# SCUT-BIP-Lab/SplatCo

Measured on AMD Instinct MI355X. Metric: rasterizer fwd+bwd Msplats/s @1080p; PSNR-match vs ref, higher is better.
Workload: dtype f32; 1 GPU; cfg1: 1M synthetic Gaussians (seed 0), 1 view 1920x1080 per GPU, GaussianRasterizer forward+backward, colors_precomp + scale/rotation path; gaussians=1000000, image=1920x1080, visible=1000000, parallelism=1 view per GPU (mv sharding)

## Files before the change

splatco_amd/csrc/binning.hip:

```cpp
#include "common.h"

namespace scr {

template <int THREADS>
__device__ __forceinline__ uint32_t block_exclusive_scan(uint32_t v, uint32_t* lds_waves ,
                                                         uint32_t& block_total) {
    const int lane = threadIdx.x & (WAVE - 1), w = threadIdx.x / WAVE;
    uint32_t inc = v;
#pragma unroll
    for (int d = 1; d < WAVE; d <<= 1) {
        uint32_t n = __shfl_up(inc, d, WAVE);
        if (lane >= d) inc += n;
    }
    if (lane == WAVE - 1) lds_waves[w] = inc;
    __syncthreads();
    uint32_t base = 0, tot = 0;
#pragma unroll
    for (int k = 0; k < THREADS / WAVE; ++k) {
        uint32_t s = lds_waves[k];
        if (k < w) base += s;
        tot += s;
    }
    block_total = tot;
    __syncthreads();
    return base + inc - v;
}

__global__ void __launch_bounds__(1024) plan_scan_kernel(uint32_t nblk, uint32_t* __restrict__ block_sums,
                                                         unsigned long long* __restrict__ total,
                                                         uint32_t tiles, const uint32_t* __restrict__ tile_count,
                                                         uint32_t* __restrict__ ranges,
                                                         uint32_t* __restrict__ cursor,
                                                         volatile unsigned long long* mailbox,
                                                         unsigned long long seq) {
    __shared__ uint32_t lds[1024 / WAVE + 1];
    __shared__ unsigned long long wide[1024 / WAVE];
    if (blockIdx.x == 0) {
        unsigned long long carry = 0, mine = 0;
        for (uint32_t base = 0; base < nblk; base += 1024) {
            uint32_t i = base + threadIdx.x;
            uint32_t v = i < nblk ? block_sums[i] : 0u, tot;
            uint32_t ex = block_exclusive_scan<1024>(v, lds, tot);
            if (i < nblk) block_sums[i] = (uint32_t)carry + ex;
            carry += tot;
            mine += v;
        }
#pragma unroll
        for (int d = WAVE / 2; d > 0; d >>= 1) mine += (unsigned long long)__shfl_down((long long)mine, d, WAVE);
        __syncthreads();
        if ((threadIdx.x & (WAVE - 1)) == 0) wide[threadIdx.x / WAVE] = mine;
        __syncthreads();
        if (threadIdx.x == 0) {
            carry = 0;
            for (int w = 0; w < 1024 / WAVE; ++w) carry += wide[w];
            total[0] = carry;
            if (mailbox) {
                mailbox[0] = carry;
                __threadfence_system();
                mailbox[1] = seq;
            }
        }
    } else {
        uint32_t carry = 0, mx = 0;
        for (uint32_t base = 0; base < tiles; base += 1024) {
            uint32_t i = base + threadIdx.x;
            uint32_t v = i < tiles ? tile_count[i] : 0u, tot;
            uint32_t ex = block_exclusive_scan<1024>(v, lds, tot);
            if (i < tiles) {
                ranges[2 * i] = carry + ex;
                ranges[2 * i + 1] = carry + ex + v;
                cursor[i] = 0;
            }
            carry += tot;
            mx = max(mx, v);
        }
#pragma unroll
        for (int d = 32; d > 0; d >>= 1) mx = max(mx, (uint32_t)__shfl_xor((int)mx, d, WAVE));
        __syncthreads();
        if ((threadIdx.x & 63) == 0) lds[threadIdx.x >> 6] = mx;
        __syncthreads();
        if (threadIdx.x == 0) {
            uint32_t m = 0;
            for (int w = 0; w < 1024 / WAVE; ++w) m = max(m, lds[w]);
            total[1] = m;
            total[2] = 0;
            if (mailbox) {
                mailbox[2] = (unsigned long long)m | (total[3] << 32);
                __threadfence_system();
                mailbox[3] = seq;
            }
        }
    }
}

template <bool LDS_HIST>
__global__ void __launch_bounds__(BIN_THREADS)
scatter_kernel(int64_t P, int gx, int tiles, const float4* __restrict__ rec, uint2* __restrict__ gm_base,
               uint32_t* __restrict__ live_bits, const uint32_t* __restrict__ tiles_touched, const uint32_t* __restrict__ block_prefix,
               uint32_t* __restrict__ point_offsets, const uint32_t* __restrict__ ranges,
               uint32_t* __restrict__ cursor, unsigned long long* __restrict__ keys,
               const unsigned long long* __restrict__ total, unsigned long long cap_instances) {
    extern __shared__ __attribute__((aligned(16))) uint32_t hist[];
    __shared__ uint32_t lds[BIN_THREADS / WAVE + 1];
    if (total[0] > cap_instances) return;
    if (LDS_HIST) {
        for (int t = threadIdx.x; t < tiles; t += BIN_THREADS) hist[t] = 0;
        __syncthreads();
    }
    uint32_t off[BIN_ROUNDS], tts[BIN_ROUNDS], rlo[BIN_ROUNDS], rhi[BIN_ROUNDS], dbits[BIN_ROUNDS];
    uint32_t carry = block_prefix[blockIdx.x];
#pragma unroll
    for (int r = 0; r < BIN_ROUNDS; ++r) {
        const int64_t i = (int64_t)blockIdx.x * BIN_GPW + r * BIN_THREADS + threadIdx.x;
        const uint32_t tt = i < P ? tiles_touched[i] : 0u;
        uint32_t tot;
        off[r] = carry + block_exclusive_scan<BIN_THREADS>(tt, lds, tot);
        carry += tot;
        tts[r] = tt;
        rlo[r] = rhi[r] = dbits[r] = 0;
        if (i < P) point_offsets[i] = off[r] + tt;
        if (tt) {
            const float4 r2 = rec[3 * i + 2];
            dbits[r] = __float_as_uint(r2.y);
            rlo[r] = __float_as_uint(r2.z);
            rhi[r] = __float_as_uint(r2.w);
            const uint32_t x0 = rlo[r] & 0xffff, y0 = rlo[r] >> 16, rw = (rhi[r] & 0xffff) - x0;
            gm_base[i] = make_uint2(off[r] - y0 * rw - x0, rw);
            if (LDS_HIST)
                for (int ty = rlo[r] >> 16; ty < (int)(rhi[r] >> 16); ++ty)
                    for (int tx = rlo[r] & 0xffff; tx < (int)(rhi[r] & 0xffff); ++tx) atomicAdd(&hist[ty * gx + tx], 1u);
        }
    }
    if (LDS_HIST) {
        __syncthreads();
        for (int t = threadIdx.x; t < tiles; t += BIN_THREADS) {
            const uint32_t c = hist[t];
            if (c) hist[t] = ranges[2 * t] + atomicAdd(&cursor[t], c);
        }
        __syncthreads();
    }
#pragma unroll
    for (int r = 0; r < BIN_ROUNDS; ++r) {
        if (!tts[r]) continue;
        const int64_t i = (int64_t)blockIdx.x * BIN_GPW + r * BIN_THREADS + threadIdx.x;
        const uint32_t klo = (uint32_t)i << 4;
        const float4 r0 = rec[3 * i], r1 = rec[3 * i + 1];
        const unsigned long long khi = (unsigned long long)dbits[r] << 32;
        uint32_t live = 0, kbit = 1;
        for (int ty = rlo[r] >> 16; ty < (int)(rhi[r] >> 16); ++ty)
            for (int tx = rlo[r] & 0xffff; tx < (int)(rhi[r] & 0xffff); ++tx) {
                const uint32_t t = (uint32_t)(ty * gx + tx);
                const uint32_t slot = LDS_HIST ? atomicAdd(&hist[t], 1u) : ranges[2 * t] + atomicAdd(&cursor[t], 1u);
                const uint32_t qm = quadrant_mask(r0, r1, tx * TILE, ty * TILE);
                keys[slot] = khi | klo | qm;
                live |= qm ? kbit : 0u;
                kbit <<= 1;
            }
        live_bits[i] = live;
    }
}

template <int D>
__device__ __forceinline__ uint32_t lane_xor(uint32_t v) {
    if constexpr (D == 1) {
        return (uint32_t)__builtin_amdgcn_mov_dpp((int)v, 0xB1, 0xf, 0xf, true);
    } else if constexpr (D == 2) {
        return (uint32_t)__builtin_amdgcn_mov_dpp((int)v, 0x4E, 0xf, 0xf, true);
    } else if constexpr (D == 4) {
        int t = __builtin_amdgcn_update_dpp((int)v, (int)v, 0x104, 0xf, 0x5, false);
        return (uint32_t)__builtin_amdgcn_update_dpp(t, (int)v, 0x114, 0xf, 0xA, false);
    } else if constexpr (D == 8) {
        int t = __builtin_amdgcn_update_dpp((int)v, (int)v, 0x108, 0xf, 0x3, false);
        return (uint32_t)__builtin_amdgcn_update_dpp(t, (int)v, 0x118, 0xf, 0xC, false);
    } else if constexpr (D == 16) {
        auto r = __builtin_amdgcn_permlane16_swap(v, v, false, false);
        return sel(0xFFFF0000FFFF0000ull, r[0], r[1]);
    } else {
        auto r = __builtin_amdgcn_permlane32_swap(v, v, false, false);
        return sel(0xFFFFFFFF00000000ull, r[0], r[1]);
    }
}

constexpr unsigned long long lanes_with_bit_clear(int bit) {
    unsigned long long m = 0;
    for (int l = 0; l < 64; ++l)
        if ((l & bit) == 0) m |= 1ull << l;
    return m;
}

template <int E, int K, int J>
__device__ __forceinline__ void bitonic_step(uint32_t (&klo)[E], uint32_t (&khi)[E], int lane) {
    if constexpr (J < E) {
#pragma unroll
        for (int e = 0; e < E; ++e) {
            if ((e & J) != 0) continue;
            const int f = e | J;
            const unsigned long long desc = K < E ? ((e & K) == 0 ? 0ull : ~0ull) : ~lanes_with_bit_clear(K / E);
            const unsigned long long a = ((unsigned long long)khi[e] << 32) | klo[e];
            const unsigned long long b = ((unsigned long long)khi[f] << 32) | klo[f];
            const unsigned long long swm = lanes(a > b) ^ desc;
            const uint32_t t0 = klo[e], t1 = khi[e];
            klo[e] = sel(swm, klo[f], t0); khi[e] = sel(swm, khi[f], t1);
            klo[f] = sel(swm, t0, klo[f]); khi[f] = sel(swm, t1, khi[f]);
        }
    } else {
        constexpr int D = J / E;
        constexpr unsigned long long keep_max = lanes_with_bit_clear(D) ^ lanes_with_bit_clear(K / E);
#pragma unroll
        for (int e = 0; e < E; ++e) {
            const uint32_t olo = lane_xor<D>(klo[e]), ohi = lane_xor<D>(khi[e]);
            const unsigned long long mine = ((unsigned long long)khi[e] << 32) | klo[e];
            const unsigned long long theirs = ((unsigned long long)ohi << 32) | olo;
            const unsigned long long take = lanes(theirs < mine) ^ keep_max;
            klo[e] = sel(take, olo, klo[e]);
            khi[e] = sel(take, ohi, khi[e]);
        }
    }
}

template <int E, int K, int J>
__device__ __forceinline__ void bitonic_stage(uint32_t (&klo)[E], uint32_t (&khi)[E], int lane) {
    bitonic_step<E, K, J>(klo, khi, lane);
    if constexpr (J > 1) bitonic_stage<E, K, J / 2>(klo, khi, lane);
}
template <int E, int K>
__device__ __forceinline__ void bitonic_network(uint32_t (&klo)[E], uint32_t (&khi)[E], int lane) {
    bitonic_stage<E, K, K / 2>(klo, khi, lane);
    if constexpr (K < 64 * E) bitonic_network<E, K * 2>(klo, khi, lane);
}

constexpr int WAVE_SORT_MAX = 1024;

struct FinalLists {
    const uint2* gm_base;
    uint32_t* point_list;
    uint32_t* gm_index;
    uint8_t* qmask;
    int tx, ty;
    __device__ __forceinline__ void write(uint32_t i, uint32_t klo) const {
        const uint32_t id = klo >> 4;
        point_list[i] = id;
        qmask[i] = (uint8_t)(klo & 15u);
        if (gm_index) {
            const uint2 b = gm_base[id];
            gm_index[i] = b.x + (uint32_t)ty * b.y + (uint32_t)tx;
        }
    }
    template <int U, typename GetK>
    __device__ __forceinline__ void write_batch(uint32_t lo, uint32_t e0, uint32_t stride, uint32_t cnt, GetK getk) const {
        uint32_t k[U];
        uint2 b[U];
#pragma unroll
        for (int u = 0; u < U; ++u) {
            const uint32_t e = e0 + (uint32_t)u * stride;
            k[u] = e < cnt ? getk(e, u) : 0u;
        }
        if (gm_index) {
#pragma unroll
            for (int u = 0; u < U; ++u) b[u] = gm_base[k[u] >> 4];
        }
        __builtin_amdgcn_sched_barrier(0);
#pragma unroll
        for (int u = 0; u < U; ++u) {
            const uint32_t e = e0 + (uint32_t)u * stride;
            if (e < cnt) {
                point_list[lo + e] = k[u] >> 4;
                qmask[lo + e] = (uint8_t)(k[u] & 15u);
                if (gm_index) gm_index[lo + e] = b[u].x + (uint32_t)ty * b[u].y + (uint32_t)tx;
            }
        }
    }
};

template <int E>
__device__ __forceinline__ void wave_sort_regs(uint32_t n, const unsigned long long* __restrict__ keys,
                                               uint32_t (&klo)[E], uint32_t (&khi)[E]) {
    const int lane = threadIdx.x & 63;
#pragma unroll
    for (int e = 0; e < E; ++e) {
        const uint32_t i = (uint32_t)e * 64 + lane;
        const unsigned long long v = i < n ? keys[i] : ~0ull;
        klo[e] = (uint32_t)v;
        khi[e] = (uint32_t)(v >> 32);
    }
    bitonic_network<E, 2>(klo, khi, lane);
}

template <int E, bool FINAL>
__device__ __forceinline__ void wave_sort(uint32_t n, unsigned long long* __restrict__ keys, uint32_t lo,
                                          const FinalLists& fl, uint32_t* __restrict__ tr) {
    const int lane = threadIdx.x & 63;
    uint32_t klo[E], khi[E];
    wave_sort_regs<E>(n, keys, klo, khi);
    auto transpose = [&](uint32_t (&w)[E]) {
        __syncthreads();
#pragma unroll
        for (int e = 0; e < E; ++e) tr[lane * (E + 1) + e] = w[e];
        __syncthreads();
#pragma unroll
        for (int e = 0; e < E; ++e) {
            const int p = e * 64 + lane;
            w[e] = tr[p + p / E];
        }
    };
    transpose(klo);
    if (!FINAL) transpose(khi);
    if (FINAL) {
        fl.template write_batch<E>(lo, (uint32_t)lane, 64u, n, [&](uint32_t, int u) { return klo[u]; });
    } else {
#pragma unroll
        for (int e = 0; e < E; ++e) {
            const uint32_t i = (uint32_t)e * 64 + lane;
            if (i < n) keys[i] = ((unsigned long long)khi[e] << 32) | klo[e];
        }
    }
}

__device__ __forceinline__ int split_slot(int p) { return p + (p >> 3); }
constexpr int SPLIT_SLOTS = WAVE_SORT_MAX + WAVE_SORT_MAX / 8;
template <int EA, int EB>
__device__ __forceinline__ void wave_sort_split(uint32_t n, const unsigned long long* __restrict__ keys, uint32_t lo,
                                                const FinalLists& fl, unsigned long long* __restrict__ mb) {
    constexpr int NA = 64 * EA, NB = 64 * EB, PER = EA + EB;
    const int lane = threadIdx.x & 63;
    {
        uint32_t klo[EA], khi[EA];
        wave_sort_regs<EA>(NA, keys, klo, khi);
#pragma unroll
        for (int e = 0; e < EA; ++e) mb[split_slot(lane * EA + e)] = ((unsigned long long)khi[e] << 32) | klo[e];
    }
    {
        uint32_t klo[EB], khi[EB];
        wave_sort_regs<EB>(n - NA, keys + NA, klo, khi);
#pragma unroll
        for (int e = 0; e < EB; ++e) mb[split_slot(NA + lane * EB + e)] = ((unsigned long long)khi[e] << 32) | klo[e];
    }
    __syncthreads();
    uint32_t outk[PER];
    {
        auto keyA = [&](uint32_t i) { return mb[split_slot((int)i)]; };
        auto keyB = [&](uint32_t j) { return mb[split_slot(NA + (int)j)]; };
        const uint32_t d0 = (uint32_t)lane * PER;
        uint32_t a = d0 > (uint32_t)NB ? d0 - NB : 0u, b = min(d0, (uint32_t)NA);
        while (a < b) {
            const uint32_t mid = (a + b) >> 1;
            if (keyA(mid) < keyB(d0 - mid - 1)) a = mid + 1;
            else b = mid;
        }
        uint32_t ia = a, ib = d0 - a;
        unsigned long long x = ia < (uint32_t)NA ? keyA(ia) : ~0ull, y = ib < (uint32_t)NB ? keyB(ib) : ~0ull;
#pragma unroll
        for (int k = 0; k < PER; ++k) {
            const bool takeA = x <= y;
            outk[k] = (uint32_t)(takeA ? x : y);
            if (takeA) {
                ++ia;
                x = ia < (uint32_t)NA ? keyA(ia) : ~0ull;
            } else {
                ++ib;
                y = ib < (uint32_t)NB ? keyB(ib) : ~0ull;
            }
        }
    }
    __syncthreads();
    uint32_t* tr = (uint32_t*)mb;
#pragma unroll
    for (int k = 0; k < PER; ++k) tr[lane * (PER + 1) + k] = outk[k];
    __syncthreads();
    fl.template write_batch<PER>(lo, (uint32_t)lane, 64u, n, [&](uint32_t i, int) { return tr[i + i / PER]; });
}

template <bool FINAL>
__device__ __forceinline__ void wave_sort_any(uint32_t n, unsigned long long* keys, uint32_t lo, const FinalLists& fl,
                                              unsigned long long* mb) {
    uint32_t* tr = (uint32_t*)mb;
    if (n <= 64) wave_sort<1, FINAL>(n, keys, lo, fl, tr);
    else if (n <= 128) wave_sort<2, FINAL>(n, keys, lo, fl, tr);
    else if (n <= 256) wave_sort<4, FINAL>(n, keys, lo, fl, tr);
    else if (FINAL && n > 256 && n <= 320) wave_sort_split<4, 1>(n, keys, lo, fl, mb);
    else if (FINAL && n > 256 && n <= 384) wave_sort_split<4, 2>(n, keys, lo, fl, mb);
    else if (n <= 512) wave_sort<8, FINAL>(n, keys, lo, fl, tr);
    else if (FINAL && n <= 576) wave_sort_split<8, 1>(n, keys, lo, fl, mb);
    else if (FINAL && n <= 640) wave_sort_split<8, 2>(n, keys, lo, fl, mb);
    else if (FINAL && n <= 768) wave_sort_split<8, 4>(n, keys, lo, fl, mb);
    else if (FINAL) wave_sort_split<8, 8>(n, keys, lo, fl, mb);
    else wave_sort<16, FINAL>(n, keys, lo, fl, tr);
}

__global__ void __launch_bounds__(64, 1)
tile_sort_wave_kernel(int tiles, int gx, const uint32_t* __restrict__ ranges, unsigned long long* __restrict__ keys,
                      const uint2* __restrict__ gm_base, uint32_t* __restrict__ point_list,
                      uint32_t* __restrict__ gm_index, uint8_t* __restrict__ qmask) {
    int t = xcd_tile(blockIdx.x, tiles);
    if (t < 0) return;
    const uint32_t lo = ranges[2 * t], n = ranges[2 * t + 1] - lo;
    if (n == 0 || n > (uint32_t)WAVE_SORT_MAX) return;
    const FinalLists fl{gm_base, point_list, gm_index, qmask, t % gx, t / gx};
    __shared__ unsigned long long mb[SPLIT_SLOTS];
    wave_sort_any<true>(n, keys + lo, lo, fl, mb);
}

constexpr int WG_SORT_THREADS = WG_SORT_MAX / 16;
__device__ __forceinline__ int wg_slot(int p) { return p + (p >> 4); }
__global__ void __launch_bounds__(WG_SORT_THREADS)
tile_sort_wg_kernel(int tiles, int gx, const uint32_t* __restrict__ ranges, unsigned long long* __restrict__ keys,
                    const uint2* __restrict__ gm_base, uint32_t* __restrict__ point_list,
                    uint32_t* __restrict__ gm_index, uint8_t* __restrict__ qmask) {
    extern __shared__ __attribute__((aligned(16))) unsigned long long buf[];
    int t = xcd_tile(blockIdx.x, tiles);
    if (t < 0) return;
    const uint32_t lo = ranges[2 * t], n = ranges[2 * t + 1] - lo;
    if (n <= (uint32_t)WAVE_SORT_MAX) return;
    const uint32_t c0 = blockIdx.y * (uint32_t)WG_SORT_MAX;
    if (c0 >= n) return;
    const uint32_t cnt = min((uint32_t)WG_SORT_MAX, n - c0);
    const int wave = threadIdx.x >> 6, lane = threadIdx.x & 63;
    unsigned long long* chunk = keys + lo + c0;
    {
        const uint32_t w0 = (uint32_t)wave * WAVE_SORT_MAX;
        const uint32_t wn = w0 < cnt ? min((uint32_t)WAVE_SORT_MAX, cnt - w0) : 0u;
        uint32_t klo[16], khi[16];
        wave_sort_regs<16>(wn, chunk + w0, klo, khi);
#pragma unroll
        for (int e = 0; e < 16; ++e)
            buf[wg_slot((int)w0 + lane * 16 + e)] = ((unsigned long long)khi[e] << 32) | klo[e];
    }
    __syncthreads();
    for (uint32_t L = WAVE_SORT_MAX; L < (uint32_t)WG_SORT_MAX && L < cnt; L <<= 1) {
        constexpr int PER = WG_SORT_MAX / WG_SORT_THREADS;
        unsigned long long outk[PER];
        const uint32_t o0 = threadIdx.x * PER, pairbase = o0 / (2u * L) * (2u * L), d0 = o0 - pairbase;
        {
            auto keyA = [&](uint32_t i) { return buf[wg_slot((int)(pairbase + i))]; };
            auto keyB = [&](uint32_t j) { return buf[wg_slot((int)(pairbase + L + j))]; };
            uint32_t a = d0 > L ? d0 - L : 0u, b = min(d0, L);
            while (a < b) {
                const uint32_t mid = (a + b) >> 1;
                if (keyA(mid) < keyB(d0 - mid - 1)) a = mid + 1;
                else b = mid;
            }
            uint32_t ia = a, ib = d0 - a;
            unsigned long long x = ia < L ? keyA(ia) : ~0ull, y = ib < L ? keyB(ib) : ~0ull;
#pragma unroll
            for (int k = 0; k < PER; ++k) {
                const bool takeA = x <= y;
                outk[k] = takeA ? x : y;
                if (takeA) {
                    ++ia;
                    x = ia < L ? keyA(ia) : ~0ull;
                } else {
                    ++ib;
                    y = ib < L ? keyB(ib) : ~0ull;
                }
            }
        }
        __syncthreads();
#pragma unroll
        for (int k = 0; k < PER; ++k) buf[wg_slot((int)(o0 + k))] = outk[k];
        __syncthreads();
    }
    const unsigned long long* src = buf;
    if (n <= (uint32_t)WG_SORT_MAX) {
        const FinalLists fl{gm_base, point_list, gm_index, qmask, t % gx, t / gx};
        for (uint32_t e = threadIdx.x; e < cnt; e += 4 * WG_SORT_THREADS)
            fl.template write_batch<4>(lo, e, (uint32_t)WG_SORT_THREADS, cnt, [&](uint32_t i, int) { return (uint32_t)src[wg_slot((int)i)]; });
    } else {
        for (uint32_t e = threadIdx.x; e < cnt; e += WG_SORT_THREADS) chunk[e] = src[wg_slot((int)e)];
    }
}

constexpr int MP_SEG = 4096;
__device__ __forceinline__ uint32_t merge_passes_needed(uint32_t n) {
    uint32_t chunks = (n + WG_SORT_MAX - 1) / WG_SORT_MAX, p = 0;
    while ((1u << p) < chunks) ++p;
    return p;
}

__device__ __forceinline__ uint32_t merge_path_cut(const unsigned long long* __restrict__ A, uint32_t la,
                                                   const unsigned long long* __restrict__ B, uint32_t lb, uint32_t s) {
    const uint32_t lane = threadIdx.x & 63;
    uint32_t lo = s > lb ? s - lb : 0u, hi = min(s, la);
    while (lo < hi) {
        const uint32_t span = hi - lo;
        const uint32_t p = span >= 65u ? lo + (uint32_t)(((unsigned long long)span * (lane + 1)) / 65u) : min(lo + lane, hi - 1);
        const bool below = A[p] < B[s - p - 1];
        const unsigned long long bal = __builtin_amdgcn_ballot_w64(below);
        const int c = __builtin_popcountll(bal);
        const uint32_t plast = __shfl(p, c > 0 ? c - 1 : 0, 64), pfirst = __shfl(p, c < 64 ? c : 63, 64);
        const uint32_t nlo = c > 0 ? plast + 1 : lo, nhi = c < 64 ? pfirst : hi;
        if (span < 65u) {
            return c < (int)min(span, 64u) ? lo + (uint32_t)c : hi;
        }
        lo = nlo;
        hi = nhi;
    }
    return lo;
}

__global__ void __launch_bounds__(256)
tile_merge_path_kernel(int tiles, int gx, uint32_t pass, const uint32_t* __restrict__ ranges,
                       const unsigned long long* __restrict__ src, unsigned long long* __restrict__ dst,
                       const uint2* __restrict__ gm_base, uint32_t* __restrict__ point_list,
                       uint32_t* __restrict__ gm_index, uint8_t* __restrict__ qmask) {
    __shared__ unsigned long long buf[MP_SEG + MP_SEG / 16];
    __shared__ uint32_t cut[2];
    int t = xcd_tile(blockIdx.x, tiles);
    if (t < 0) return;
    const uint32_t lo = ranges[2 * t], n = ranges[2 * t + 1] - lo;
    if (n <= (uint32_t)WG_SORT_MAX || pass >= merge_passes_needed(n)) return;
    const uint32_t L = (uint32_t)WG_SORT_MAX << pass;
    const uint32_t e0 = blockIdx.y * (uint32_t)MP_SEG;
    if (e0 >= n) return;
    const uint32_t pairbase = e0 / (2u * L) * (2u * L);
    const uint32_t lenA = min(L, n - pairbase);
    const uint32_t lenB = n - pairbase > L ? min(L, n - pairbase - L) : 0u;
    const uint32_t s0 = e0 - pairbase, s1 = min(s0 + (uint32_t)MP_SEG, lenA + lenB);
    const unsigned long long* A = src + lo + pairbase;
    const unsigned long long* B = A + L;
    if (threadIdx.x < 128) {
        const int w = threadIdx.x >> 6;
        const uint32_t cw = merge_path_cut(A, lenA, B, lenB, w ? s1 : s0);
        if ((threadIdx.x & 63) == 0) cut[w] = cw;
    }
    __syncthreads();
    const uint32_t i0 = cut[0], na = cut[1] - i0, j0 = s0 - i0, nb = (s1 - s0) - na;
    const uint32_t tot = na + nb;
    {
        unsigned long long v[MP_SEG / 256];
#pragma unroll
        for (int k = 0; k < MP_SEG / 256; ++k) {
            const uint32_t e = min(threadIdx.x + 256u * k, tot - 1);
            v[k] = e < na ? A[i0 + e] : B[j0 + (e - na)];
        }
#pragma unroll
        for (int k = 0; k < MP_SEG / 256; ++k) {
            const uint32_t e = threadIdx.x + 256u * k;
            if (e < tot) buf[wg_slot((int)e)] = v[k];
        }
    }
    __syncthreads();
    constexpr int PER = MP_SEG / 256;
    unsigned long long outk[PER];
    const uint32_t d0 = min((uint32_t)threadIdx.x * PER, tot);
    {
        auto keyA = [&](uint32_t i) { return buf[wg_slot((int)i)]; };
        auto keyB = [&](uint32_t j) { return buf[wg_slot((int)(na + j))]; };
        uint32_t a = d0 > nb ? d0 - nb : 0u, b = min(d0, na);
        while (a < b) {
            const uint32_t mid = (a + b) >> 1;
            if (keyA(mid) < keyB(d0 - mid - 1)) a = mid + 1;
            else b = mid;
        }
        uint32_t ia = a, ib = d0 - a;
        unsigned long long x = ia < na ? keyA(ia) : ~0ull, y = ib < nb ? keyB(ib) : ~0ull;
#pragma unroll
        for (int k = 0; k < PER; ++k) {
            const bool takeA = x < y;
            outk[k] = takeA ? x : y;
            if (takeA) {
                ++ia;
                x = ia < na ? keyA(ia) : ~0ull;
            } else {
                ++ib;
                y = ib < nb ? keyB(ib) : ~0ull;
            }
        }
    }
    __syncthreads();
#pragma unroll
    for (int k = 0; k < PER; ++k)
        if (d0 + k < tot) buf[wg_slot((int)(d0 + k))] = outk[k];
    __syncthreads();
    if (pass + 1 == merge_passes_needed(n)) {
        const FinalLists fl{gm_base, point_list, gm_index, qmask, t % gx, t / gx};
        for (uint32_t e = threadIdx.x; e < tot; e += 4 * 256)
            fl.template write_batch<4>(lo + pairbase + s0, e, 256u, tot, [&](uint32_t i, int) { return (uint32_t)buf[wg_slot((int)i)]; });
    } else {
        unsigned long long* out = dst + lo + pairbase + s0;
        for (uint32_t e = threadIdx.x; e < tot; e += 256) out[e] = buf[wg_slot((int)e)];
    }
}

void launch_plan_scans(int64_t P, const KSettings& ks, const GeomView& gv, unsigned long long* mailbox,
                       unsigned long long seq, hipStream_t st) {
    Grid g(ks.H, ks.W);
    uint32_t nb = (uint32_t)((P + BIN_GPW - 1) / BIN_GPW);
    plan_scan_kernel<<<2, 1024, 0, st>>>(nb, gv.block_sums, gv.total, (uint32_t)g.tiles, gv.tile_count,
                                         gv.ranges, gv.cursor, mailbox, seq);
}

void launch_scatter(int64_t P, const KSettings& ks, const GeomView& gv, const BinView& bv, unsigned long long cap_instances,
                    hipStream_t st) {
    if (P <= 0) return;
    Grid g(ks.H, ks.W);
    const unsigned nb = (unsigned)((P + BIN_GPW - 1) / BIN_GPW);
    allow_dynamic_lds((const void*)scatter_kernel<true>, LDS_HIST_MAX_TILES * 4);
    if (g.tiles <= LDS_HIST_MAX_TILES)
        scatter_kernel<true><<<nb, BIN_THREADS, (size_t)g.tiles * 4, st>>>(
            P, g.gx, g.tiles, gv.rec, gv.gm_base, gv.live_bits, gv.tiles_touched, gv.block_sums, gv.point_offsets, gv.ranges,
            gv.cursor, bv.keys, gv.total, cap_instances);
    else
        scatter_kernel<false><<<nb, BIN_THREADS, 0, st>>>(
            P, g.gx, g.tiles, gv.rec, gv.gm_base, gv.live_bits, gv.tiles_touched, gv.block_sums, gv.point_offsets, gv.ranges,
            gv.cursor, bv.keys, gv.total, cap_instances);
}

void launch_tile_sort(const KSettings& ks, const GeomView& gv, const BinView& bv, int64_t max_tile_instances,
                      bool with_gm_index, hipStream_t st) {
    uint32_t* const gm_index = with_gm_index ? bv.gm_index : nullptr;
    Grid g(ks.H, ks.W);
    const unsigned gt = (unsigned)xcd_grid(g.tiles);
    if (max_tile_instances <= 0) return;
    tile_sort_wave_kernel<<<gt, 64, 0, st>>>(g.tiles, g.gx, gv.ranges, bv.keys, gv.gm_base, bv.point_list, gm_index,
                                             bv.qmask);
    if (max_tile_instances <= WAVE_SORT_MAX) return;
    const unsigned chunks = (unsigned)((max_tile_instances + WG_SORT_MAX - 1) / WG_SORT_MAX);
    const size_t lds = (size_t)(WG_SORT_MAX + WG_SORT_MAX / 16) * 8;
    allow_dynamic_lds((const void*)tile_sort_wg_kernel, lds);
    tile_sort_wg_kernel<<<dim3(gt, chunks), WG_SORT_THREADS, lds, st>>>(g.tiles, g.gx, gv.ranges, bv.keys, gv.gm_base, bv.point_list,
                                                                        gm_index, bv.qmask);
    if (chunks <= 1) return;
    unsigned passes = 0;
    while ((1u << passes) < chunks) ++passes;
    const unsigned segs = (unsigned)((max_tile_instances + MP_SEG - 1) / MP_SEG);
    for (unsigned p = 0; p < passes; ++p) {
        const unsigned long long* src = (p & 1u) ? bv.keys2 : bv.keys;
        unsigned long long* dst = (p & 1u) ? bv.keys : bv.keys2;
        tile_merge_path_kernel<<<dim3(gt, segs), 256, 0, st>>>(g.tiles, g.gx, p, gv.ranges, src, dst, gv.gm_base,
                                                               bv.point_list, gm_index, bv.qmask);
    }
}

}
```

Baseline: 1096 Msplats/s.

## Use f64 min/max bitonic compare-exchange with mirror stages and vectorized scan

Replaces the register bitonic sort's 64-bit compare plus select on split lo/hi halves with v_min_f64/v_max_f64 on packed keys. This relies on keys below a padding value ordering the same way as doubles. The network is reworked to use mirror (flip) stages, so every lane does min or max under an exec mask with no direction masks, and cheaper DPP and swizzle lane permutes replace permlane16. The plan scan kernel also processes 8 elements per thread with uint4 loads and stores. The risks are NaN or denormal handling in the f64 ops on key bit patterns and the use of inline asm that rewrites exec.

```diff
diff --git a/splatco_amd/csrc/binning.hip b/splatco_amd/csrc/binning.hip
--- a/splatco_amd/csrc/binning.hip
+++ b/splatco_amd/csrc/binning.hip
@@ -26,6 +26,20 @@
     return base + inc - v;
 }
 
+constexpr int SCAN_PER = 8;
+constexpr uint32_t SCAN_CHUNK = 1024u * SCAN_PER;
+__device__ __forceinline__ bool aligned16(const void* p) { return ((uintptr_t)p & 15u) == 0; }
+__device__ __forceinline__ void scan_load(const uint32_t* __restrict__ src, uint32_t i0, uint32_t n, bool vec,
+                                          uint32_t (&v)[SCAN_PER]) {
+    if (vec && i0 < n && n - i0 >= (uint32_t)SCAN_PER) {
+        const uint4 a = *(const uint4*)(src + i0), b = *(const uint4*)(src + i0 + 4);
+        v[0] = a.x; v[1] = a.y; v[2] = a.z; v[3] = a.w;
+        v[4] = b.x; v[5] = b.y; v[6] = b.z; v[7] = b.w;
+    } else {
+#pragma unroll
+        for (int k = 0; k < SCAN_PER; ++k) v[k] = i0 < n && (uint32_t)k < n - i0 ? src[i0 + k] : 0u;
+    }
+}
 __global__ void __launch_bounds__(1024) plan_scan_kernel(uint32_t nblk, uint32_t* __restrict__ block_sums,
                                                          unsigned long long* __restrict__ total,
                                                          uint32_t tiles, const uint32_t* __restrict__ tile_count,
@@ -35,15 +49,31 @@
                                                          unsigned long long seq) {
     __shared__ uint32_t lds[1024 / WAVE + 1];
     __shared__ unsigned long long wide[1024 / WAVE];
+    static_assert(SCAN_PER == 8, "scan_load and the stores below move two uint4 per thread");
     if (blockIdx.x == 0) {
         unsigned long long carry = 0, mine = 0;
-        for (uint32_t base = 0; base < nblk; base += 1024) {
-            uint32_t i = base + threadIdx.x;
-            uint32_t v = i < nblk ? block_sums[i] : 0u, tot;
-            uint32_t ex = block_exclusive_scan<1024>(v, lds, tot);
-            if (i < nblk) block_sums[i] = (uint32_t)carry + ex;
+        const bool vec = aligned16(block_sums);
+        for (uint32_t base = 0; base < nblk; base += SCAN_CHUNK) {
+            const uint32_t i0 = base + threadIdx.x * SCAN_PER;
+            uint32_t v[SCAN_PER], sum = 0, tot;
+            scan_load(block_sums, i0, nblk, vec, v);
+#pragma unroll
+            for (int k = 0; k < SCAN_PER; ++k) {
+                const uint32_t x = v[k];
+                mine += x;
+                v[k] = sum;
+                sum += x;
+            }
+            const uint32_t ex = (uint32_t)carry + block_exclusive_scan<1024>(sum, lds, tot);
+            if (vec && i0 < nblk && nblk - i0 >= (uint32_t)SCAN_PER) {
+                *(uint4*)(block_sums + i0) = make_uint4(ex + v[0], ex + v[1], ex + v[2], ex + v[3]);
+                *(uint4*)(block_sums + i0 + 4) = make_uint4(ex + v[4], ex + v[5], ex + v[6], ex + v[7]);
+            } else {
+#pragma unroll
+                for (int k = 0; k < SCAN_PER; ++k)
+                    if (i0 < nblk && (uint32_t)k < nblk - i0) block_sums[i0 + k] = ex + v[k];
+            }
             carry += tot;
-            mine += v;
         }
 #pragma unroll
         for (int d = WAVE / 2; d > 0; d >>= 1) mine += (unsigned long long)__shfl_down((long long)mine, d, WAVE);
@@ -62,17 +92,41 @@
         }
     } else {
         uint32_t carry = 0, mx = 0;
-        for (uint32_t base = 0; base < tiles; base += 1024) {
-            uint32_t i = base + threadIdx.x;
-            uint32_t v = i < tiles ? tile_count[i] : 0u, tot;
-            uint32_t ex = block_exclusive_scan<1024>(v, lds, tot);
-            if (i < tiles) {
-                ranges[2 * i] = carry + ex;
-                ranges[2 * i + 1] = carry + ex + v;
-                cursor[i] = 0;
+        const bool vec = aligned16(tile_count) && aligned16(ranges) && aligned16(cursor);
+        for (uint32_t base = 0; base < tiles; base += SCAN_CHUNK) {
+            const uint32_t i0 = base + threadIdx.x * SCAN_PER;
+            uint32_t v[SCAN_PER], sum = 0, tot;
+            scan_load(tile_count, i0, tiles, vec, v);
+#pragma unroll
+            for (int k = 0; k < SCAN_PER; ++k) {
+                mx = max(mx, v[k]);
+                sum += v[k];
+            }
+            uint32_t s = carry + block_exclusive_scan<1024>(sum, lds, tot);
+            if (vec && i0 < tiles && tiles - i0 >= (uint32_t)SCAN_PER) {
+                uint32_t e[SCAN_PER + 1];
+                e[0] = s;
+#pragma unroll
+                for (int k = 0; k < SCAN_PER; ++k) e[k + 1] = e[k] + v[k];
+                uint4* r = (uint4*)(ranges + 2 * (size_t)i0);
+                r[0] = make_uint4(e[0], e[1], e[1], e[2]);
+                r[1] = make_uint4(e[2], e[3], e[3], e[4]);
+                r[2] = make_uint4(e[4], e[5], e[5], e[6]);
+                r[3] = make_uint4(e[6], e[7], e[7], e[8]);
+                *(uint4*)(cursor + i0) = make_uint4(0, 0, 0, 0);
+                *(uint4*)(cursor + i0 + 4) = make_uint4(0, 0, 0, 0);
+            } else {
+#pragma unroll
+                for (int k = 0; k < SCAN_PER; ++k) {
+                    if (i0 < tiles && (uint32_t)k < tiles - i0) {
+                        ranges[2 * (size_t)(i0 + k)] = s;
+                        ranges[2 * (size_t)(i0 + k) + 1] = s + v[k];
+                        cursor[i0 + k] = 0;
+                    }
+                    s += v[k];
+                }
             }
             carry += tot;
-            mx = max(mx, v);
         }
 #pragma unroll
         for (int d = 32; d > 0; d >>= 1) mx = max(mx, (uint32_t)__shfl_xor((int)mx, d, WAVE));
@@ -167,18 +221,42 @@
     } else if constexpr (D == 2) {
         return (uint32_t)__builtin_amdgcn_mov_dpp((int)v, 0x4E, 0xf, 0xf, true);
     } else if constexpr (D == 4) {
-        int t = __builtin_amdgcn_update_dpp((int)v, (int)v, 0x104, 0xf, 0x5, false);
-        return (uint32_t)__builtin_amdgcn_update_dpp(t, (int)v, 0x114, 0xf, 0xA, false);
+        const int t = __builtin_amdgcn_mov_dpp((int)v, 0x141, 0xf, 0xf, true);
+        return (uint32_t)__builtin_amdgcn_mov_dpp(t, 0x1B, 0xf, 0xf, true);
     } else if constexpr (D == 8) {
-        int t = __builtin_amdgcn_update_dpp((int)v, (int)v, 0x108, 0xf, 0x3, false);
-        return (uint32_t)__builtin_amdgcn_update_dpp(t, (int)v, 0x118, 0xf, 0xC, false);
+        const int t = __builtin_amdgcn_mov_dpp((int)v, 0x140, 0xf, 0xf, true);
+        return (uint32_t)__builtin_amdgcn_mov_dpp(t, 0x141, 0xf, 0xf, true);
     } else if constexpr (D == 16) {
-        auto r = __builtin_amdgcn_permlane16_swap(v, v, false, false);
-        return sel(0xFFFF0000FFFF0000ull, r[0], r[1]);
+        return (uint32_t)__builtin_amdgcn_ds_swizzle((int)v, 0x401F);
     } else {
         auto r = __builtin_amdgcn_permlane32_swap(v, v, false, false);
         return sel(0xFFFFFFFF00000000ull, r[0], r[1]);
     }
+}
+template <int M>
+__device__ __forceinline__ uint32_t lane_mirror(uint32_t v) {
+    if constexpr (M == 1) {
+        return lane_xor<1>(v);
+    } else if constexpr (M == 3) {
+        return (uint32_t)__builtin_amdgcn_mov_dpp((int)v, 0x1B, 0xf, 0xf, true);
+    } else if constexpr (M == 7) {
+        return (uint32_t)__builtin_amdgcn_mov_dpp((int)v, 0x141, 0xf, 0xf, true);
+    } else if constexpr (M == 15) {
+        return (uint32_t)__builtin_amdgcn_mov_dpp((int)v, 0x140, 0xf, 0xf, true);
+    } else if constexpr (M == 31) {
+        return (uint32_t)__builtin_amdgcn_ds_swizzle((int)v, 0x7C1F);
+    } else {
+        static_assert(M == 63, "lane_mirror: M = 2^k - 1 <= 63");
+        return lane_xor<32>(lane_mirror<31>(v));
+    }
+}
+template <int D>
+__device__ __forceinline__ unsigned long long lane_xor64(unsigned long long v) {
+    return ((unsigned long long)lane_xor<D>((uint32_t)(v >> 32)) << 32) | lane_xor<D>((uint32_t)v);
+}
+template <int M>
+__device__ __forceinline__ unsigned long long lane_mirror64(unsigned long long v) {
+    return ((unsigned long long)lane_mirror<M>((uint32_t)(v >> 32)) << 32) | lane_mirror<M>((uint32_t)v);
 }
 
 constexpr unsigned long long lanes_with_bit_clear(int bit) {
@@ -188,45 +266,92 @@
     return m;
 }
 
+constexpr unsigned long long SORT_PAD = 0x7FEFFFFFFFFFFFFFull;
+__device__ __forceinline__ unsigned long long kmin(unsigned long long a, unsigned long long b) {
+    unsigned long long r;
+    asm("v_min_f64 %0, %1, %2" : "=v"(r) : "v"(a), "v"(b));
+    return r;
+}
+__device__ __forceinline__ unsigned long long kmax(unsigned long long a, unsigned long long b) {
+    unsigned long long r;
+    asm("v_max_f64 %0, %1, %2" : "=v"(r) : "v"(a), "v"(b));
+    return r;
+}
+
+#define SCR_KEEP_MIN(a, b) "v_min_f64 %" #a ", %" #a ", %" #b "\n\t"
+#define SCR_KEEP_MAX(a, b) "v_max_f64 %" #a ", %" #a ", %" #b "\n\t"
+template <int G>
+__device__ __forceinline__ void keep_minmax(unsigned long long minmask, unsigned long long* k, const unsigned long long* o) {
+    if constexpr (G == 1) {
+        asm volatile("s_mov_b64 exec, %2\n\t" SCR_KEEP_MIN(0, 1) "s_not_b64 exec, exec\n\t" SCR_KEEP_MAX(0, 1) "s_mov_b64 exec, -1"
+                     : "+v"(k[0]) : "v"(o[0]), "s"(minmask) : "scc");
+    } else if constexpr (G == 2) {
+        asm volatile("s_mov_b64 exec, %4\n\t" SCR_KEEP_MIN(0, 2) SCR_KEEP_MIN(1, 3) "s_not_b64 exec, exec\n\t"
+                     SCR_KEEP_MAX(0, 2) SCR_KEEP_MAX(1, 3) "s_mov_b64 exec, -1"
+                     : "+v"(k[0]), "+v"(k[1]) : "v"(o[0]), "v"(o[1]), "s"(minmask) : "scc");
+    } else if constexpr (G == 4) {
+        asm volatile("s_mov_b64 exec, %8\n\t" SCR_KEEP_MIN(0, 4) SCR_KEEP_MIN(1, 5) SCR_KEEP_MIN(2, 6) SCR_KEEP_MIN(3, 7)
+                     "s_not_b64 exec, exec\n\t" SCR_KEEP_MAX(0, 4) SCR_KEEP_MAX(1, 5) SCR_KEEP_MAX(2, 6) SCR_KEEP_MAX(3, 7)
+                     "s_mov_b64 exec, -1"
+                     : "+v"(k[0]), "+v"(k[1]), "+v"(k[2]), "+v"(k[3])
+                     : "v"(o[0]), "v"(o[1]), "v"(o[2]), "v"(o[3]), "s"(minmask) : "scc");
+    } else {
+        static_assert(G == 8, "keep_minmax: groups of 1, 2, 4 or 8 exchanges");
+        asm volatile("s_mov_b64 exec, %16\n\t" SCR_KEEP_MIN(0, 8) SCR_KEEP_MIN(1, 9) SCR_KEEP_MIN(2, 10) SCR_KEEP_MIN(3, 11)
+                     SCR_KEEP_MIN(4, 12) SCR_KEEP_MIN(5, 13) SCR_KEEP_MIN(6, 14) SCR_KEEP_MIN(7, 15) "s_not_b64 exec, exec\n\t"
+                     SCR_KEEP_MAX(0, 8) SCR_KEEP_MAX(1, 9) SCR_KEEP_MAX(2, 10) SCR_KEEP_MAX(3, 11) SCR_KEEP_MAX(4, 12)
+                     SCR_KEEP_MAX(5, 13) SCR_KEEP_MAX(6, 14) SCR_KEEP_MAX(7, 15) "s_mov_b64 exec, -1"
+                     : "+v"(k[0]), "+v"(k[1]), "+v"(k[2]), "+v"(k[3]), "+v"(k[4]), "+v"(k[5]), "+v"(k[6]), "+v"(k[7])
+                     : "v"(o[0]), "v"(o[1]), "v"(o[2]), "v"(o[3]), "v"(o[4]), "v"(o[5]), "v"(o[6]), "v"(o[7]), "s"(minmask)
+                     : "scc");
+    }
+}
+#undef SCR_KEEP_MIN
+#undef SCR_KEEP_MAX
+
 template <int E, int K, int J>
-__device__ __forceinline__ void bitonic_step(uint32_t (&klo)[E], uint32_t (&khi)[E], int lane) {
-    if constexpr (J < E) {
+__device__ __forceinline__ void bitonic_step(unsigned long long (&k)[E]) {
+    constexpr bool MIRROR = J == 0;
+    constexpr int DIST = MIRROR ? K / 2 : J;
+    if constexpr (DIST < E) {
 #pragma unroll
         for (int e = 0; e < E; ++e) {
-            if ((e & J) != 0) continue;
-            const int f = e | J;
-            const unsigned long long desc = K < E ? ((e & K) == 0 ? 0ull : ~0ull) : ~lanes_with_bit_clear(K / E);
-            const unsigned long long a = ((unsigned long long)khi[e] << 32) | klo[e];
-            const unsigned long long b = ((unsigned long long)khi[f] << 32) | klo[f];
-            const unsigned long long swm = lanes(a > b) ^ desc;
-            const uint32_t t0 = klo[e], t1 = khi[e];
-            klo[e] = sel(swm, klo[f], t0); khi[e] = sel(swm, khi[f], t1);
-            klo[f] = sel(swm, t0, klo[f]); khi[f] = sel(swm, t1, khi[f]);
-        }
-    } else {
-        constexpr int D = J / E;
-        constexpr unsigned long long keep_max = lanes_with_bit_clear(D) ^ lanes_with_bit_clear(K / E);
-#pragma unroll
-        for (int e = 0; e < E; ++e) {
-            const uint32_t olo = lane_xor<D>(klo[e]), ohi = lane_xor<D>(khi[e]);
-            const unsigned long long mine = ((unsigned long long)khi[e] << 32) | klo[e];
-            const unsigned long long theirs = ((unsigned long long)ohi << 32) | olo;
-            const unsigned long long take = lanes(theirs < mine) ^ keep_max;
-            klo[e] = sel(take, olo, klo[e]);
-            khi[e] = sel(take, ohi, khi[e]);
+            if ((e & DIST) != 0) continue;
+            const int f = MIRROR ? (e ^ (K - 1)) : (e | J);
+            const unsigned long long lo = kmin(k[e], k[f]), hi = kmax(k[e], k[f]);
+            k[e] = lo;
+            k[f] = hi;
+        }
+    } else {
+        constexpr unsigned long long minmask = lanes_with_bit_clear(DIST / E);
+        constexpr int G = E < 8 ? E : 8;
+#pragma unroll
+        for (int g0 = 0; g0 < E; g0 += G) {
+            auto idx = [&](int g) { return !MIRROR ? g0 + g : g < G / 2 ? g0 / 2 + g : E - 1 - (g0 / 2 + g - G / 2); };
+            unsigned long long kk[G], o[G];
+#pragma unroll
+            for (int g = 0; g < G; ++g) {
+                kk[g] = k[idx(g)];
+                if constexpr (MIRROR) o[g] = lane_mirror64<K / E - 1>(k[idx(g) ^ (E - 1)]);
+                else o[g] = lane_xor64<J / E>(k[idx(g)]);
+            }
+            keep_minmax<G>(minmask, kk, o);
+#pragma unroll
+            for (int g = 0; g < G; ++g) k[idx(g)] = kk[g];
         }
     }
 }
 
 template <int E, int K, int J>
-__device__ __forceinline__ void bitonic_stage(uint32_t (&klo)[E], uint32_t (&khi)[E], int lane) {
-    bitonic_step<E, K, J>(klo, khi, lane);
-    if constexpr (J > 1) bitonic_stage<E, K, J / 2>(klo, khi, lane);
+__device__ __forceinline__ void bitonic_stage(unsigned long long (&k)[E]) {
+    bitonic_step<E, K, J>(k);
+    if constexpr (J > 1) bitonic_stage<E, K, J / 2>(k);
 }
 template <int E, int K>
-__device__ __forceinline__ void bitonic_network(uint32_t (&klo)[E], uint32_t (&khi)[E], int lane) {
-    bitonic_stage<E, K, K / 2>(klo, khi, lane);
-    if constexpr (K < 64 * E) bitonic_network<E, K * 2>(klo, khi, lane);
+__device__ __forceinline__ void bitonic_network(unsigned long long (&k)[E]) {
+    bitonic_step<E, K, 0>(k);
+    if constexpr (K >= 4) bitonic_stage<E, K, K / 4>(k);
+    if constexpr (K < 64 * E) bitonic_network<E, K * 2>(k);
 }
 
 constexpr int WAVE_SORT_MAX = 1024;
@@ -274,24 +399,28 @@
 
 template <int E>
 __device__ __forceinline__ void wave_sort_regs(uint32_t n, const unsigned long long* __restrict__ keys,
-                                               uint32_t (&klo)[E], uint32_t (&khi)[E]) {
+                                               unsigned long long (&k)[E]) {
     const int lane = threadIdx.x & 63;
 #pragma unroll
     for (int e = 0; e < E; ++e) {
         const uint32_t i = (uint32_t)e * 64 + lane;
-        const unsigned long long v = i < n ? keys[i] : ~0ull;
-        klo[e] = (uint32_t)v;
-        khi[e] = (uint32_t)(v >> 32);
-    }
-    bitonic_network<E, 2>(klo, khi, lane);
+        k[e] = i < n ? keys[i] : SORT_PAD;
+    }
+    bitonic_network<E, 2>(k);
 }
 
 template <int E, bool FINAL>
 __device__ __forceinline__ void wave_sort(uint32_t n, unsigned long long* __restrict__ keys, uint32_t lo,
                                           const FinalLists& fl, uint32_t* __restrict__ tr) {
     const int lane = threadIdx.x & 63;
+    unsigned long long k[E];
+    wave_sort_regs<E>(n, keys, k);
     uint32_t klo[E], khi[E];
-    wave_sort_regs<E>(n, keys, klo, khi);
+#pragma unroll
+    for (int e = 0; e < E; ++e) {
+        klo[e] = (uint32_t)k[e];
+        khi[e] = (uint32_t)(k[e] >> 32);
+    }
     auto transpose = [&](uint32_t (&w)[E]) {
         __syncthreads();
 #pragma unroll
@@ -324,16 +453,16 @@
     constexpr int NA = 64 * EA, NB = 64 * EB, PER = EA + EB;
     const int lane = threadIdx.x & 63;
     {
-        uint32_t klo[EA], khi[EA];
-        wave_sort_regs<EA>(NA, keys, klo, khi);
-#pragma unroll
-        for (int e = 0; e < EA; ++e) mb[split_slot(lane * EA + e)] = ((unsigned long long)khi[e] << 32) | klo[e];
+        unsigned long long k[EA];
+        wave_sort_regs<EA>(NA, keys, k);
+#pragma unroll
+        for (int e = 0; e < EA; ++e) mb[split_slot(lane * EA + e)] = k[e];
     }
     {
-        uint32_t klo[EB], khi[EB];
-        wave_sort_regs<EB>(n - NA, keys + NA, klo, khi);
-#pragma unroll
-        for (int e = 0; e < EB; ++e) mb[split_slot(NA + lane * EB + e)] = ((unsigned long long)khi[e] << 32) | klo[e];
+        unsigned long long k[EB];
+        wave_sort_regs<EB>(n - NA, keys + NA, k);
+#pragma unroll
+        for (int e = 0; e < EB; ++e) mb[split_slot(NA + lane * EB + e)] = k[e];
     }
     __syncthreads();
     uint32_t outk[PER];
@@ -419,11 +548,10 @@
     {
         const uint32_t w0 = (uint32_t)wave * WAVE_SORT_MAX;
         const uint32_t wn = w0 < cnt ? min((uint32_t)WAVE_SORT_MAX, cnt - w0) : 0u;
-        uint32_t klo[16], khi[16];
-        wave_sort_regs<16>(wn, chunk + w0, klo, khi);
-#pragma unroll
-        for (int e = 0; e < 16; ++e)
-            buf[wg_slot((int)w0 + lane * 16 + e)] = ((unsigned long long)khi[e] << 32) | klo[e];
+        unsigned long long k[16];
+        wave_sort_regs<16>(wn, chunk + w0, k);
+#pragma unroll
+        for (int e = 0; e < 16; ++e) buf[wg_slot((int)w0 + lane * 16 + e)] = k[e];
     }
     __syncthreads();
     for (uint32_t L = WAVE_SORT_MAX; L < (uint32_t)WG_SORT_MAX && L < cnt; L <<= 1) {
```

Result: no change. 1107 Msplats/s, median of 6 (+1.0%).
